# pakozm/lua-mapreduce

Hardware: AMD Instinct MI355X
Metric: words/sec (higher is better)
Workload: dtype u8-text/i64-counts; 1 GPU; model=europarl-wordcount, global_batch=49158635, seq_len=49158635, parallelism=dp1, splits_per_gpu=197, partitions=1, partitioner=hash-mulhi, ingestion=resident-hbm

## Files before the change

mapreduce_amd/ops/hip/mr_kernels.hip:

```cpp

#include "common.h"


#define TOK_BYTES 16

__global__ void tokenize_kernel(const u8* __restrict__ text, long n,
                                u64* __restrict__ out_hash,
                                u64* __restrict__ out_pos,
                                unsigned long long* __restrict__ counter,
                                long cap) {
  long t0 = ((long)blockIdx.x * blockDim.x + threadIdx.x) * (long)TOK_BYTES;
  long stride = (long)gridDim.x * blockDim.x * TOK_BYTES;
  for (long base = t0; base < n; base += stride) {
    long end = base + TOK_BYTES < n ? base + TOK_BYTES : n;
    u8 prev = (base == 0) ? ' ' : text[base - 1];
    for (long i = base; i < end; ++i) {
      u8 c = text[i];
      if (!is_ws(c) && is_ws(prev)) {
        u64 h = FNV64_OFFSET;
        long j = i;
        while (j < n) {
          u8 cc = text[j];
          if (is_ws(cc)) break;
          h ^= cc;
// ... 697 lines not shown
        int lane = threadIdx.x & (WAVE - 1);
        unsigned long long lt_mask =
            (lane == 63) ? ~0ull >> 1 : ((1ull << lane) - 1);
        while (pending) {
          int leader = __ffsll(pending) - 1;
          u64 lead_bk = __shfl(bk, leader, WAVE);
          unsigned long long members =
              __ballot(mine && bk == lead_bk) & pending;
          int nmem = __popcll(members);
          unsigned long long base = 0;
          if (lane == leader)
            base = atomicAdd(&spill_counter[lead_bk],
                             (unsigned long long)nmem);
          base = __shfl(base, leader, WAVE);
          if (members & (1ull << lane)) {
            long r = (long)base + __popcll(members & lt_mask);
            if (r < spill_cap) {
              long o = (long)lead_bk * spill_cap + r;
              out_hash[o] = sh_[wi];
              out_pos[o] = mypos;
            }
          }
          pending &= ~members;
        }
      }
    } else {
      u32 my_ns = (u32)__popc(miss_mask);
      u32 incl = my_ns;
      #pragma unroll
      for (int off = 1; off < WAVE; off <<= 1) {
        u32 x = __shfl_up(incl, off, WAVE);
        if ((threadIdx.x & (WAVE - 1)) >= off) incl += x;
      }
      u32 wave_total = __shfl(incl, WAVE - 1, WAVE);
      int lane = threadIdx.x & (WAVE - 1);
      if (wave_total && (int)wave_total > wleft) {
        for (int i = lane; i < wleft; i += WAVE)
          if (wchunk + i < spill_cap) out_hash[wchunk + i] = HT_EMPTY;
        int grab = (int)wave_total > SPILL_CHUNK ? (int)wave_total
                                                 : SPILL_CHUNK;
        unsigned long long nb = 0;
        if (lane == 0)
          nb = atomicAdd(spill_counter, (unsigned long long)grab);
        wchunk = (long)__shfl(nb, 0, WAVE);
        wleft = grab;
      }
      long o = wchunk + (long)(incl - my_ns);
      if (wave_total) {
        wchunk += wave_total;
        wleft -= (int)wave_total;
      }
      u32 smw = sm0;
      #pragma unroll
      for (int wi = 0; wi < 8; ++wi) {
        if (miss_mask & (1u << wi)) {
          u64 p = v6_spill_pos(wpos0, smw, m32, long_len);
          if (MODE == 4) {
            my_words += sh_[wi] + p + (u64)o;
          } else if (o < spill_cap) {
            out_hash[o] = sh_[wi];
            out_pos[o] = p;
          }
          ++o;
        }
        smw &= smw - 1;
      }
    }
    }
  }
  {
    int lane = threadIdx.x & (WAVE - 1);
    for (int i = lane; i < wleft; i += WAVE)
      if (wchunk + i < spill_cap) out_hash[wchunk + i] = HT_EMPTY;
  }
  __syncthreads();
  for (int s = tid; s < CACHE_N; s += blockDim.x)
    if (ckeys[s] != HT_EMPTY && ccnt[s])
      ht_add(ckeys[s], cpos[s], (i64)ccnt[s], tkeys, tvals, texm, cap_mask);
  unsigned long long ws = my_words;
  for (int off = 32; off > 0; off >>= 1) ws += __shfl_down(ws, off, WAVE);
  if (lane_id() == 0 && ws) atomicAdd(nwords, ws);
}

__global__ __launch_bounds__(256) void tok_ablate_kernel(
    const u8* __restrict__ text, long n, int mode,
    u64* __restrict__ ckeys_g , i64* __restrict__ sink,
    u64* __restrict__ out_hash, u64* __restrict__ out_pos,
    unsigned long long* __restrict__ spill_counter, long spill_cap) {
  __shared__ u8 tile[TOK_TILE + TOK_HALO];
  __shared__ u64 ckeys[TOK_CACHE];
  __shared__ u64 cpos[TOK_CACHE];
  __shared__ u32 ccnt[TOK_CACHE];
  for (int s = threadIdx.x; s < TOK_CACHE; s += blockDim.x) {
    ckeys[s] = HT_EMPTY;
    ccnt[s] = 0;
  }
  unsigned long long acc = 0;
  long tile0 = (long)blockIdx.x * TOK_TILE;
  long tstride = (long)gridDim.x * TOK_TILE;
  for (long base = tile0; base < n; base += tstride) {
    __syncthreads();
    long avail = n - base;
    long want = avail < TOK_TILE + TOK_HALO ? avail : TOK_TILE + TOK_HALO;
    for (int o = threadIdx.x * 16; o < want; o += blockDim.x * 16) {
      if (o + 16 <= want && (((uintptr_t)&text[base + o]) & 15) == 0) {
        *(uint4*)&tile[o] = *(const uint4*)&text[base + o];
      } else {
        for (int b = 0; b < 16 && o + b < want; ++b)
          tile[o + b] = text[base + o + b];
      }
    }
    __syncthreads();
    if (mode == 1) {
      acc += tile[threadIdx.x];
      continue;
    }
    long my0 = (long)threadIdx.x * TOK_BYTES;
    long myend = my0 + TOK_BYTES;
    if (myend > avail) myend = avail;
    if (my0 >= myend) continue;
    u64 sh[8];
    u64 sp[8];
    int ns = 0;
    u8 prev = (base + my0 == 0) ? ' ' : (my0 ? tile[my0 - 1] : text[base - 1]);
    for (long i = my0; i < myend; ++i) {
      u8 c = tile[i];
      if (!is_ws(c) && is_ws(prev)) {
        u64 h = FNV64_OFFSET;
        long j = i;
        if (mode == 2) {
          while (j < want && !is_ws(tile[j])) ++j;
          acc += (u64)(j - i);
        } else {
          while (j < want) {
            u8 cc = tile[j];
            if (is_ws(cc)) break;
            h ^= cc;
            h *= FNV64_PRIME;
            ++j;
          }
          if (j == want && base + j < n) {
            long g = base + j;
            while (g < n && !is_ws(text[g])) {
              h ^= text[g];
              h *= FNV64_PRIME;
              ++g;
            }
            j = g - base;
          }
        }
        if (mode == 3) {
          acc += h;
        } else if (mode >= 4) {
          u64 k = remap_key(h);
          u64 p = ((u64)(base + i) << 16) | (u64)(j - i);
          u32 slot = (u32)((k ^ (k >> 32)) & (TOK_CACHE - 1));
          bool done = false;
          for (int pr = 0; pr < TOK_PROBE; ++pr) {
            u64 cur = ckeys[slot];
            if (cur == k) {
              atomicAdd(&ccnt[slot], 1u);
              done = true;
              break;
            }
            if (cur == HT_EMPTY) {
              u64 prevk = atomicCAS((unsigned long long*)&ckeys[slot],
// ... 385 lines not shown
```

mapreduce_amd/ops/hip/ops_ext.hip:

```cpp

#include <ATen/hip/HIPContext.h>
#include <torch/extension.h>

#include <limits>
#include <map>
#include <mutex>
#include <optional>
#include <utility>

#include "asof.hip"
#include "extract_sorted.hip"
#include "frame.hip"
#include "gradsum.hip"
#include "graph.hip"
#include "group.hip"
#include "join.hip"
#include "lex_order.hip"
#include "mr_kernels.hip"
#include "postings_phrase.hip"
#include "postings_query.hip"
#include "radix_sort.hip"
#include "seg_scan.hip"
#include "token_ordinals.hip"

namespace {

constexpr int kBlock = 256;
constexpr long kMaxBlocks = 2048;

long grid_for(long n, long per_thread = 1) {
  long want = (n + (long)kBlock * per_thread - 1) / ((long)kBlock * per_thread);
  if (want < 1) want = 1;
  return want < kMaxBlocks ? want : kMaxBlocks;
}

hipStream_t cur_stream() { return at::hip::getCurrentHIPStream(); }

constexpr int kTokWavesPerCu = 16;

struct TokOccupancy {
  int blocks_per_cu = 0;
  int cus = 0;
};

TokOccupancy tok_occupancy(const void* kfn, int blockn) {
  static std::mutex mu;
  static std::map<std::pair<const void*, int>, TokOccupancy> cache;
  int dev = 0;
  C10_HIP_CHECK(hipGetDevice(&dev));
  std::lock_guard<std::mutex> lock(mu);
  auto it = cache.find({kfn, dev});
  if (it != cache.end()) return it->second;
  TokOccupancy o;
  C10_HIP_CHECK(hipOccupancyMaxActiveBlocksPerMultiprocessor(
      &o.blocks_per_cu, kfn, blockn, 0));
  C10_HIP_CHECK(hipDeviceGetAttribute(
      &o.cus, hipDeviceAttributeMultiprocessorCount, dev));
  TORCH_CHECK(o.blocks_per_cu > 0 && o.cus > 0,
              "tokenizer occupancy query returned ", o.blocks_per_cu,
              " blocks/CU on ", o.cus, " CUs");
  cache[{kfn, dev}] = o;
  return o;
}

template <typename K>
long tok_grid(K kfn, int blockn, long n, long tile_bytes) {
  long tiles = (n + tile_bytes - 1) / tile_bytes;
  if (tiles < 1) tiles = 1;
  TokOccupancy o = tok_occupancy(reinterpret_cast<const void*>(kfn), blockn);
  int per_cu = kTokWavesPerCu / (blockn / WAVE);
  if (per_cu > o.blocks_per_cu) per_cu = o.blocks_per_cu;
  long resident = (long)per_cu * o.cus;
  long blocks = tiles < resident ? tiles : resident;
  return blocks < kMaxBlocks ? blocks : kMaxBlocks;
}

int rs_items() {
  static int v = -1;
  if (v < 0) {
    const char* e = getenv("MR_RS_ITEMS");
    const char* v1 = getenv("MR_RADIX_V1");
    v = (e && atoi(e) == 4 && !(v1 && v1[0] == '1')) ? 4 : 8;
  }
  return v;
}

long rs_tile() { return (long)RS_BLOCK * rs_items(); }

bool radix_v1_forced() {
  const char* v = getenv("MR_RADIX_V1");
  return v && v[0] == '1';
}

bool radix_v2_forced() {
  static int f = -1;
  if (f < 0) {
    const char* v = getenv("MR_RADIX_V2");
    f = (v && v[0] == '1') ? 1 : 0;
  }
  return f == 1;
}

#define RS_STAGED_SCATTER(VT, SKIP, BT, LATE)                              \
  (radix_v2_forced()                                                       \
       ? (rs_items() == 4 ? radix_scatter_v2_kernel<4, VT, SKIP, BT>       \
                          : radix_scatter_v2_kernel<8, VT, SKIP, BT>)      \
       : (rs_items() == 4 ? radix_scatter_v3_kernel<4, VT, SKIP, BT, LATE> \
                          : radix_scatter_v3_kernel<8, VT, SKIP, BT, LATE>))

void launch_radix_hist(const u64* kin, long n, int shift, long ntiles,
                       i64* hist) {
  auto kfn = rs_items() == 4 ? radix_hist_kernel<4> : radix_hist_kernel<8>;
  hipLaunchKernelGGL(kfn, dim3(ntiles), dim3(RS_BLOCK), 0, cur_stream(),
                     kin, n, shift, ntiles, hist);
}

void launch_radix_scatter(const u64* kin, const u64* vin, long n, int shift,
                          long ntiles, const i64* base, u64* kout,
                          u64* vout) {
  static int use_v1 = -1;
  if (use_v1 < 0) use_v1 = radix_v1_forced() ? 1 : 0;
  if (use_v1)
    hipLaunchKernelGGL(radix_scatter_kernel, dim3(ntiles), dim3(RS_BLOCK), 0,
                       cur_stream(), kin, vin, n, shift, ntiles, base, kout,
                       vout);
  else {
    auto kfn = RS_STAGED_SCATTER(u64, false, i64, true);
    hipLaunchKernelGGL(kfn, dim3(ntiles), dim3(RS_BLOCK),
                       0, cur_stream(), kin, vin, n, shift, ntiles, base,
                       kout, vout);
  }
}

void launch_radix_scatter32(const u64* kin, const u32* vin, long n,
                            int shift, long ntiles, const i64* base,
                            u64* kout, u32* vout) {
  auto kfn = RS_STAGED_SCATTER(u32, false, i64, true);
  hipLaunchKernelGGL(kfn, dim3(ntiles), dim3(RS_BLOCK), 0, cur_stream(),
                     kin, vin, n, shift, ntiles, base, kout, vout);
}

template <bool SKIP>
void launch_bucketize_hist(const u64* kin, long n, int shift, long ntiles,
                           u32* hist) {
  auto kfn = rs_items() == 4 ? radix_hist_kernel<4, SKIP, u32, true>
                             : radix_hist_kernel<8, SKIP, u32, true>;
  if (radix_v2_forced())
    kfn = rs_items() == 4 ? radix_hist_kernel<4, SKIP, u32>
                          : radix_hist_kernel<8, SKIP, u32>;
  hipLaunchKernelGGL(kfn, dim3(ntiles), dim3(RS_BLOCK), 0, cur_stream(),
                     kin, n, shift, ntiles, hist);
}

template <typename VT, bool SKIP>
void launch_bucketize_scatter(const u64* kin, const VT* vin, long n,
                              int shift, long ntiles, const u32* base,
                              u64* kout, VT* vout) {
  auto kfn = RS_STAGED_SCATTER(VT, SKIP, u32, false);
  hipLaunchKernelGGL(kfn, dim3(ntiles), dim3(RS_BLOCK), 0, cur_stream(),
                     kin, vin, n, shift, ntiles, base, kout, vout);
}

u64* u64p(torch::Tensor& t) { return reinterpret_cast<u64*>(t.data_ptr<i64>()); }
const u64* u64cp(const torch::Tensor& t) {
  return reinterpret_cast<const u64*>(t.data_ptr<i64>());
}

void check_dev_i64(const torch::Tensor& t, const char* name) {
  TORCH_CHECK(t.is_cuda(), name, " must be on GPU");
  TORCH_CHECK(t.scalar_type() == torch::kInt64, name, " must be int64");
  TORCH_CHECK(t.is_contiguous(), name, " must be contiguous");
}

}

std::vector<torch::Tensor> tokenize(torch::Tensor text, long cap) {
  TORCH_CHECK(text.is_cuda() && text.scalar_type() == torch::kUInt8 &&
              text.is_contiguous(), "text must be contiguous u8 on GPU");
  long n = text.numel();
  auto opts = torch::TensorOptions().device(text.device()).dtype(torch::kInt64);
  auto out_hash = torch::empty({cap}, opts);
  auto out_pos = torch::empty({cap}, opts);
  auto counter = torch::zeros({1}, opts);
  long blocks = grid_for(n, TOK_BYTES);
  hipLaunchKernelGGL(tokenize_kernel, dim3(blocks), dim3(kBlock), 0,
                     cur_stream(), text.data_ptr<u8>(), n, u64p(out_hash),
                     u64p(out_pos),
                     reinterpret_cast<unsigned long long*>(counter.data_ptr<i64>()),
                     cap);
  return {out_hash, out_pos, counter};
}

void tokenize_count(torch::Tensor text, long pos_base, torch::Tensor tkeys,
                    torch::Tensor tvals, torch::Tensor texm,
                    torch::Tensor nwords) {
  TORCH_CHECK(text.is_cuda() && text.scalar_type() == torch::kUInt8 &&
              text.is_contiguous(), "text must be contiguous u8 on GPU");
  long n = text.numel();
  long cap = tkeys.numel();
  TORCH_CHECK((cap & (cap - 1)) == 0, "table capacity must be a power of 2");
  if (!n) return;
  hipLaunchKernelGGL(tokenize_count_kernel, dim3(grid_for(n, TOK_BYTES)),
                     dim3(kBlock), 0, cur_stream(), text.data_ptr<u8>(), n,
                     (u64)pos_base, u64p(tkeys), tvals.data_ptr<i64>(),
                     texm.numel() ? u64p(texm) : nullptr, (u64)(cap - 1),
                     reinterpret_cast<unsigned long long*>(nwords.data_ptr<i64>()));
}

std::vector<torch::Tensor> tokenize_spill_v2(torch::Tensor text,
                                             long pos_base, long cap) {
  TORCH_CHECK(text.is_cuda() && text.scalar_type() == torch::kUInt8 &&
              text.is_contiguous(), "text must be contiguous u8 on GPU");
  long n = text.numel();
  auto opts = torch::TensorOptions().device(text.device()).dtype(torch::kInt64);
  auto out_hash = torch::empty({cap}, opts);
  auto out_pos = torch::empty({cap}, opts);
  auto counter = torch::zeros({1}, opts);
  auto nwords = torch::zeros({1}, opts);
  if (n) {
    auto dummy = torch::empty({16}, opts);
    hipLaunchKernelGGL((tokenize_v6_kernel<16, false, 4096, 0, true>),
                       dim3(grid_for(n, TOK_BYTES)), dim3(kBlock), 0,
                       cur_stream(), text.data_ptr<u8>(), n, (u64)pos_base,
                       u64p(dummy), dummy.data_ptr<i64>(), nullptr,
                       (u64)15, u64p(out_hash), u64p(out_pos),
                       reinterpret_cast<unsigned long long*>(counter.data_ptr<i64>()),
                       cap,
                       reinterpret_cast<unsigned long long*>(nwords.data_ptr<i64>()),
                       nullptr, (const i64*)nullptr, 0, 0L);
  }
  return {out_hash, out_pos, counter, nwords};
}

std::vector<torch::Tensor> tokenize_spill_composite(
    torch::Tensor text, long pos_base, long cap, torch::Tensor split_off,
    long doc_base) {
  TORCH_CHECK(text.is_cuda() && text.scalar_type() == torch::kUInt8 &&
              text.is_contiguous(), "text must be contiguous u8 on GPU");
  check_dev_i64(split_off, "split_off");
  long n = text.numel();
  auto opts = torch::TensorOptions().device(text.device()).dtype(torch::kInt64);
  auto out_hash = torch::empty({cap}, opts);
  auto out_pos = torch::empty({cap}, opts);
  auto counter = torch::zeros({1}, opts);
  auto nwords = torch::zeros({1}, opts);
  if (n) {
    auto dummy = torch::empty({16}, opts);
    hipLaunchKernelGGL((tokenize_v6_kernel<16, false, 4096, 0, true, true>),
                       dim3(grid_for(n, TOK_BYTES)), dim3(kBlock), 0,
                       cur_stream(), text.data_ptr<u8>(), n, (u64)pos_base,
                       u64p(dummy), dummy.data_ptr<i64>(), nullptr,
                       (u64)15, u64p(out_hash), u64p(out_pos),
                       reinterpret_cast<unsigned long long*>(counter.data_ptr<i64>()),
                       cap,
                       reinterpret_cast<unsigned long long*>(nwords.data_ptr<i64>()),
                       nullptr, split_off.data_ptr<i64>(),
                       (int)split_off.numel(), doc_base);
  }
  return {out_hash, out_pos, counter, nwords};
}

void tokenize_cache_spill_composite(
    torch::Tensor text, long pos_base, torch::Tensor tkeys,
    torch::Tensor tvals, torch::Tensor texm, long spill_cap,
    torch::Tensor nwords, torch::Tensor out_hash, torch::Tensor out_pos,
    torch::Tensor counter, torch::Tensor split_off, long doc_base) {
  TORCH_CHECK(text.is_cuda() && text.scalar_type() == torch::kUInt8 &&
              text.is_contiguous(), "text must be contiguous u8 on GPU");
  check_dev_i64(split_off, "split_off");
  long n = text.numel();
  long cap = tkeys.numel();
  TORCH_CHECK((cap & (cap - 1)) == 0, "table capacity must be a power of 2");
  TORCH_CHECK(out_hash.numel() >= spill_cap && out_pos.numel() >= spill_cap,
              "spill arrays too small");
  if (!n) return;
  auto kfn =
      tokenize_v6_kernel<2048, true, 4096, 0, false, true, 2048, 0, 256>;
  long blocks = tok_grid(kfn, kBlock, n, 4096);
  static torch::Tensor cpos_gc;
  long need = blocks * 2048;
  if (!cpos_gc.defined() || cpos_gc.numel() < need ||
      cpos_gc.device() != text.device())
    cpos_gc = torch::empty({need}, torch::TensorOptions()
                                        .device(text.device())
                                        .dtype(torch::kInt64));
  hipLaunchKernelGGL(
      kfn, dim3(blocks), dim3(kBlock), 0, cur_stream(), text.data_ptr<u8>(), n,
      (u64)pos_base, u64p(tkeys), tvals.data_ptr<i64>(),
      texm.numel() ? u64p(texm) : nullptr, (u64)(cap - 1), u64p(out_hash),
      u64p(out_pos),
      reinterpret_cast<unsigned long long*>(counter.data_ptr<i64>()),
      spill_cap,
      reinterpret_cast<unsigned long long*>(nwords.data_ptr<i64>()),
      u64p(cpos_gc), split_off.data_ptr<i64>(), (int)split_off.numel(),
      doc_base);
}

std::vector<torch::Tensor> tokenize_spill(torch::Tensor text, long pos_base,
                                          long cap) {
  TORCH_CHECK(text.is_cuda() && text.scalar_type() == torch::kUInt8 &&
              text.is_contiguous(), "text must be contiguous u8 on GPU");
  long n = text.numel();
  auto opts = torch::TensorOptions().device(text.device()).dtype(torch::kInt64);
  auto out_hash = torch::empty({cap}, opts);
  auto out_pos = torch::empty({cap}, opts);
  auto counter = torch::zeros({1}, opts);
  if (n)
    hipLaunchKernelGGL(tokenize_spill_kernel, dim3(grid_for(n, TOK_BYTES)),
                       dim3(kBlock), 0, cur_stream(), text.data_ptr<u8>(), n,
                       (u64)pos_base, u64p(out_hash), u64p(out_pos),
                       reinterpret_cast<unsigned long long*>(counter.data_ptr<i64>()),
                       cap);
  return {out_hash, out_pos, counter};
}

void tokenize_cache_spill(
    torch::Tensor text, long pos_base, torch::Tensor tkeys,
    torch::Tensor tvals, torch::Tensor texm, long spill_cap,
    torch::Tensor nwords, torch::Tensor out_hash, torch::Tensor out_pos,
    torch::Tensor counter) {
  TORCH_CHECK(text.is_cuda() && text.scalar_type() == torch::kUInt8 &&
              text.is_contiguous(), "text must be contiguous u8 on GPU");
  long n = text.numel();
  long cap = tkeys.numel();
  TORCH_CHECK((cap & (cap - 1)) == 0, "table capacity must be a power of 2");
  TORCH_CHECK(out_hash.numel() >= spill_cap && out_pos.numel() >= spill_cap,
              "spill arrays too small");
  if (n) {
    const char* v = getenv("MR_TOKENIZE_V5");
    const char* v4 = getenv("MR_TOKENIZE_V4");
    if (!(v && v[0] == '1') && !(v4 && v4[0] == '1')) {
      const char* cs = getenv("MR_TOK_CACHE");
      int cache = cs ? atoi(cs) : 2048;
      const char* gp = getenv("MR_TOK_GPOS");
      bool gpos = !(gp && gp[0] == '0');
      const char* ts = getenv("MR_TOK_TILE");
      int tsz = ts ? atoi(ts) : 4096;
      const char* sc = getenv("MR_SPILL_CHUNK");
      int schunk = sc ? atoi(sc) : 2048;
      const char* tb = getenv("MR_TOK_BLOCK");
      int blockn = (tb && atoi(tb) == 512) ? 512 : 256;
      if (blockn == 512) tsz = 8192;
      auto kfn = tokenize_v6_kernel<2048, false, 4096>;
      if (gpos && blockn == 512)
        kfn = tokenize_v6_kernel<2048, true, 8192, 0, false, false, 2048,
                                 0, 512>;
      else if (gpos && tsz == 8192) kfn = tokenize_v6_kernel<2048, true, 8192>;
      else if (gpos && cache == 4096) kfn = tokenize_v6_kernel<4096, true, 4096>;
      else if (gpos && cache == 1024) kfn = tokenize_v6_kernel<1024, true, 4096>;
      else if (gpos && schunk == 128)
        kfn = tokenize_v6_kernel<2048, true, 4096, 0, false, false, 128>;
      else if (gpos && schunk == 1024)
        kfn = tokenize_v6_kernel<2048, true, 4096, 0, false, false, 1024>;
      else if (gpos && schunk == 2048)
        kfn = tokenize_v6_kernel<2048, true, 4096, 0, false, false, 2048>;
      else if (gpos && schunk == 4096)
        kfn = tokenize_v6_kernel<2048, true, 4096, 0, false, false, 4096>;
      else if (gpos) kfn = tokenize_v6_kernel<2048, true, 4096>;
      else if (cache == 512) kfn = tokenize_v6_kernel<512, false, 4096>;
      else if (cache == 1024) kfn = tokenize_v6_kernel<1024, false, 4096>;
      else if (schunk == 128)
        kfn = tokenize_v6_kernel<2048, false, 4096, 0, false, false, 128>;
      long blocks = tok_grid(kfn, blockn, n, tsz);
      static torch::Tensor cpos_g;
      u64* cpg = nullptr;
      if (gpos) {
        long need = blocks * (cache > 2048 ? cache : 2048);
        if (!cpos_g.defined() || cpos_g.numel() < need ||
            cpos_g.device() != text.device())
          cpos_g = torch::empty({need},
                                torch::TensorOptions().device(text.device())
                                    .dtype(torch::kInt64));
        cpg = u64p(cpos_g);
      }
      hipLaunchKernelGGL(kfn,
                         dim3(blocks), dim3(blockn), 0,
                         cur_stream(), text.data_ptr<u8>(), n, (u64)pos_base,
                         u64p(tkeys), tvals.data_ptr<i64>(),
                         texm.numel() ? u64p(texm) : nullptr, (u64)(cap - 1),
                         u64p(out_hash), u64p(out_pos),
                         reinterpret_cast<unsigned long long*>(counter.data_ptr<i64>()),
                         spill_cap,
                         reinterpret_cast<unsigned long long*>(nwords.data_ptr<i64>()),
                         cpg, (const i64*)nullptr, 0, 0L);
    } else if (!(v && v[0] == '1'))
      hipLaunchKernelGGL(tokenize_cache_spill_kernel,
                         dim3(grid_for(n, TOK_BYTES)), dim3(kBlock), 0,
                         cur_stream(), text.data_ptr<u8>(), n, (u64)pos_base,
                         u64p(tkeys), tvals.data_ptr<i64>(),
                         texm.numel() ? u64p(texm) : nullptr, (u64)(cap - 1),
                         u64p(out_hash), u64p(out_pos),
                         reinterpret_cast<unsigned long long*>(counter.data_ptr<i64>()),
                         spill_cap,
                         reinterpret_cast<unsigned long long*>(nwords.data_ptr<i64>()));
    else
      hipLaunchKernelGGL(tokenize_v5_kernel,
                         dim3(grid_for(n, TOK_BYTES)), dim3(kBlock), 0,
                         cur_stream(), text.data_ptr<u8>(), n, (u64)pos_base,
                         u64p(tkeys), tvals.data_ptr<i64>(),
                         texm.numel() ? u64p(texm) : nullptr, (u64)(cap - 1),
                         u64p(out_hash), u64p(out_pos),
                         reinterpret_cast<unsigned long long*>(counter.data_ptr<i64>()),
                         spill_cap,
                         reinterpret_cast<unsigned long long*>(nwords.data_ptr<i64>()));
  }
}

void tokenize_cache_spill_bucketed(
    torch::Tensor text, long pos_base, torch::Tensor tkeys,
    torch::Tensor tvals, torch::Tensor texm, long spill_bcap,
    torch::Tensor nwords, torch::Tensor out_hash, torch::Tensor out_pos,
    torch::Tensor counters) {
  TORCH_CHECK(text.is_cuda() && text.scalar_type() == torch::kUInt8 &&
              text.is_contiguous(), "text must be contiguous u8 on GPU");
  long n = text.numel();
  long cap = tkeys.numel();
  TORCH_CHECK((cap & (cap - 1)) == 0, "table capacity must be a power of 2");
  TORCH_CHECK(counters.numel() >= 256, "counters must hold 256 buckets");
  TORCH_CHECK(out_hash.numel() >= 256 * spill_bcap &&
              out_pos.numel() >= 256 * spill_bcap, "spill arrays too small");
  if (!n) return;
  const char* gp = getenv("MR_TOK_GPOS");
  bool gpos = !(gp && gp[0] == '0');
  auto kfn = tokenize_v6_kernel<2048, false, 4096, 0, false, false, 512, 256>;
  if (gpos)
    kfn = tokenize_v6_kernel<2048, true, 4096, 0, false, false, 512, 256>;
  long blocks = tok_grid(kfn, kBlock, n, 4096);
  static torch::Tensor cpos_gb;
  u64* cpg = nullptr;
  if (gpos) {
    long need = blocks * 2048;
    if (!cpos_gb.defined() || cpos_gb.numel() < need ||
        cpos_gb.device() != text.device())
      cpos_gb = torch::empty({need},
                             torch::TensorOptions().device(text.device())
                                 .dtype(torch::kInt64));
    cpg = u64p(cpos_gb);
  }
  hipLaunchKernelGGL(kfn, dim3(blocks), dim3(kBlock), 0, cur_stream(),
                     text.data_ptr<u8>(), n, (u64)pos_base, u64p(tkeys),
                     tvals.data_ptr<i64>(),
                     texm.numel() ? u64p(texm) : nullptr, (u64)(cap - 1),
                     u64p(out_hash), u64p(out_pos),
                     reinterpret_cast<unsigned long long*>(counters.data_ptr<i64>()),
                     spill_bcap,
                     reinterpret_cast<unsigned long long*>(nwords.data_ptr<i64>()),
// ... 1259 lines not shown

namespace {
static_assert(GRAPH_BLOCK == SEG_SCAN_BLOCK,
              "the graph kernels are launched by SEG_SCAN_LAUNCH");

void check_graph_f64(const torch::Tensor& t, const torch::Tensor& like,
                     long n, const char* name) {
  TORCH_CHECK(t.is_cuda(), name, " must be on GPU");
  TORCH_CHECK(t.scalar_type() == torch::kFloat64, name, " must be float64");
  TORCH_CHECK(t.is_contiguous(), name, " must be contiguous");
  TORCH_CHECK(t.device() == like.device(), name,
              " must be on the device of sums");
  TORCH_CHECK(t.numel() == n, name, " must hold ", n, " entries, got ",
              t.numel());
}
}

torch::Tensor graph_propagate(torch::Tensor offsets, torch::Tensor src,
                              torch::Tensor x, long op, bool f64) {
  check_dev_i64(offsets, "offsets");
  check_dev_i64(x, "x");
  TORCH_CHECK(src.is_cuda(), "src must be on GPU");
  TORCH_CHECK(src.scalar_type() == torch::kInt32, "src must be int32");
  TORCH_CHECK(src.is_contiguous(), "src must be contiguous");
  TORCH_CHECK(offsets.device() == x.device() && src.device() == x.device(),
              "offsets, src and x must be on the same device");
  long n = x.numel(), m = src.numel();
  TORCH_CHECK(offsets.numel() == n + 1, "offsets must hold ", n + 1,
              " entries, got ", offsets.numel());
  TORCH_CHECK(n < (1L << 31) && m < (1L << 31),
              "graph ops take fewer than 2^31 edges and rows, got ", m,
              " and ", n);
  TORCH_CHECK(op >= SEG_SUM && op <= SEG_MAX,
              "op must be 0 (sum), 1 (min) or 2 (max), got ", op);
  TORCH_CHECK(op == SEG_SUM || !f64, "graph min / max take int64 values");
  const i64 ident = op == SEG_SUM ? 0
                    : op == SEG_MIN ? std::numeric_limits<i64>::max()
                                    : std::numeric_limits<i64>::min();
  auto out = torch::full({n}, ident, x.options());
  if (!n || !m) return out;
  long ntiles = (m + GRAPH_TILE - 1) / GRAPH_TILE;
  auto tf = torch::empty({ntiles}, x.options());
  auto ta = torch::empty({ntiles}, x.options());
  auto lr = torch::empty({ntiles}, x.options());
  auto la = torch::empty({ntiles}, x.options());
  SEG_SCAN_LAUNCH(graph_tile_kernel, ntiles, offsets.data_ptr<i64>(),
                  src.data_ptr<int>(), u64cp(x), n, m, u64p(out),
                  tf.data_ptr<i64>(), u64p(ta), lr.data_ptr<i64>(), u64p(la));
  auto c = seg_scan_carry(tf, ta, op, f64);
  SEG_SCAN_LAUNCH(graph_lead_kernel, grid_for(ntiles), lr.data_ptr<i64>(),
                  u64cp(la), c[0].data_ptr<i64>(), u64cp(c[1]), ntiles, n,
                  u64p(out));
  return out;
}

std::vector<torch::Tensor> pagerank_update(torch::Tensor sums,
                                           torch::Tensor old,
                                           torch::Tensor inv_out,
                                           double damping,
                                           torch::Tensor dangling) {
  long n = sums.numel();
  check_graph_f64(sums, sums, n, "sums");
  check_graph_f64(old, sums, n, "old");
  check_graph_f64(inv_out, sums, n, "inv_out");
  check_graph_f64(dangling, sums, 1, "dangling");
  TORCH_CHECK(n < (1L << 31), "graph ops take fewer than 2^31 rows, got ", n);
  auto nw = torch::empty({n}, sums.options());
  auto contrib = torch::empty({n}, sums.options());
  long blocks = n ? grid_for(n) : 0;
  if (blocks > GRAPH_PR_BLOCKS) blocks = GRAPH_PR_BLOCKS;
  auto partials = torch::empty({blocks, 2}, sums.options());
  if (blocks)
    hipLaunchKernelGGL(pagerank_update_kernel, dim3(blocks),
                       dim3(GRAPH_BLOCK), 0, cur_stream(),
                       sums.data_ptr<double>(), old.data_ptr<double>(),
                       inv_out.data_ptr<double>(), n, damping,
                       dangling.data_ptr<double>(), nw.data_ptr<double>(),
                       contrib.data_ptr<double>(),
                       partials.data_ptr<double>());
  return {nw, contrib, partials};
}

py::dict tokenizer_occupancy() {
  auto kfn = tokenize_v6_kernel<2048, true, 4096, 0, false, false, 2048>;
  TokOccupancy o = tok_occupancy(reinterpret_cast<const void*>(kfn), kBlock);
  hipFuncAttributes fa;
  C10_HIP_CHECK(hipFuncGetAttributes(&fa, reinterpret_cast<const void*>(kfn)));
  py::dict d;
  d["blocks_per_cu"] = o.blocks_per_cu;
  d["cus"] = o.cus;
  d["num_regs"] = fa.numRegs;
  d["lds_bytes"] = (long)fa.sharedSizeBytes;
  return d;
}

PYBIND11_MODULE(TORCH_EXTENSION_NAME, m) {
  m.def("group_caps", &group_caps, "(TILE, QMAX) of the group kernels");
  m.def("group_rank_max", &group_rank_max,
        "longest segment of the tile kernel's rank-counting pass");
  m.def("group_order_keys", &group_order_keys,
        "u64 order key of each i64 / f64 value");
  m.def("group_tile_sort", &group_tile_sort,
        "values ordered inside every segment that fits one tile");
  m.def("group_tile_sort_perm", &group_tile_sort_perm,
        "group_tile_sort plus the input row of every value");
  m.def("seg_scan_caps", &seg_scan_caps,
        "(TILE, CARRY_CHUNK) of the segmented scan");
  m.def("scan_by_key_sorted", &scan_by_key_sorted,
        "inclusive sum/min/max scan within runs of equal keys");
  m.def("seg_scan_reduce", &seg_scan_reduce,
        "pass 1 of scan_by_key_sorted: per-tile (flags, aggregate)");
  m.def("seg_scan_carry", &seg_scan_carry,
        "pass 2 of scan_by_key_sorted: per-tile carry-in");
  m.def("seg_scan_apply", &seg_scan_apply,
        "pass 3 of scan_by_key_sorted: the running column");
  m.def("session_flags", &session_flags,
        "1 where a row starts a key or follows a gap in time");
  m.def("graph_caps", &graph_caps,
        "(TILE, PR_BLOCKS) of the graph kernels");
  m.def("graph_propagate", &graph_propagate,
        "sum / min / max over every row's in-edges of a gathered column");
  m.def("pagerank_update", &pagerank_update,
        "one PageRank update -> (new, contrib, partials)");
  m.def("frame_caps", &frame_caps,
        "(TILE, WIN, RTILE) of the frame kernels");
  m.def("frame_bounds", &frame_bounds, py::arg("keys"), py::arg("times"),
        py::arg("preceding"), py::arg("following"), py::arg("row") = false,
        "range frames of (key, time)-sorted rows -> (lo, hi)");
  m.def("frame_reduce", &frame_reduce,
        "sum / min / max of a value column over per-row frames");
  m.def("frame_tile", &frame_tile,
        "frame_reduce pass 1: (pre, suf, tile aggregates)");
  m.def("frame_tree", &frame_tree,
        "frame_reduce pass 2: the tree over the tile aggregates");
  m.def("frame_apply", &frame_apply,
        "frame_reduce pass 3: one range query per row");
  m.def("group_pick", &group_pick,
        "values at exact rank fractions of each ordered segment");
  m.def("group_distinct_flags", &group_distinct_flags,
        "1 where a row starts a segment or a new value");
  m.def("join_bounds", &join_bounds, py::arg("lkeys"), py::arg("rkeys"),
        py::arg("window") = true,
        "(lo, cnt) of each left key in the sorted right keys");
  m.def("join_bounds_caps", &join_bounds_caps,
        "(BTILE, WIN) of the windowed join_bounds");
  m.def("join_expand", &join_expand,
        "(li, ri) row pairs from the bounds and their exclusive cumsum");
  m.def("join_caps", &join_caps, "(TILE, LDS_ROWS) of join_expand");
  m.def("asof_sorted", &asof_sorted, py::arg("lkeys"), py::arg("ltimes"),
        py::arg("rkeys"), py::arg("rtimes"), py::arg("direction") = 0,
        py::arg("tolerance") = py::none(), py::arg("allow_exact") = true,
        py::arg("f64") = false, py::arg("row") = false,
        "matched right row (or -1) of each left row of two sorted relations");
  m.def("asof_caps", &asof_caps, "(TILE, WIN) of the windowed asof_sorted");
  m.def("tokenizer_occupancy", &tokenizer_occupancy,
        "blocks/CU, registers and static LDS of the default tokenizer");
  m.def("postings_search", &postings_search,
        "ranked AND/OR top-k over the inverted index, one block per query");
  m.def("postings_search_caps", &postings_search_caps,
        "(TMAX, KMAX, BUF) of postings_search");
  m.def("postings_phrase", &postings_phrase,
        "exact-phrase top-k over the positional index, one block per query");
  m.def("token_ordinals", &token_ordinals,
        "(doc, token ordinal within doc) of each occurrence");
  m.def("token_ordinals_caps", &token_ordinals_caps,
        "(GRANULE) of token_ordinals");
  m.def("lex_chunk_keys", &lex_chunk_keys,
        "big-endian 8-byte chunk d of each string as a sortable u64");
  m.def("lex_refine", &lex_refine,
        "(seg, key) head flags + unfinished-string flags");
  m.def("lex_lower_bound", &lex_lower_bound,
        "binary search of byte-string queries in a lex permutation");
  m.def("radix_sort_idx32", &radix_sort_idx32,
        "sort u64 keys with a u32 iota payload -> (keys, perm)");
  m.def("gather_by_u32", &gather_by_u32, "out[i] = vals[idx[i]] (u32 idx)");
  m.def("tokenize", &tokenize, "tokenize text -> (hash, pos, count)");
  m.def("tokenize_count", &tokenize_count,
        "fused tokenize + hash-table count");
  m.def("tokenize_spill_composite", &tokenize_spill_composite,
        "spill-all with fused (word,doc) composite keys");
  m.def("tokenize_cache_spill_composite", &tokenize_cache_spill_composite,
        "composite keys with the LDS cache (misses spill)");
  m.def("tokenize_spill_v2", &tokenize_spill_v2,
        "spill-all tokenizer (chunk-padded; filter HT_EMPTY)");
  m.def("tokenize_spill", &tokenize_spill,
        "tokenize -> compact (hash,pos) arrays");
  m.def("tokenize_cache_spill", &tokenize_cache_spill,
        "tokenize; LDS cache counts the head, misses spill");
  m.def("tokenize_cache_spill_bucketed", &tokenize_cache_spill_bucketed,
        "tokenize; misses spill directly into per-top-byte-bucket regions");
  m.def("tok_ablate", &tok_ablate, "ablation timing (diagnosis)");
  m.def("tok6_ablate", &tok6_ablate, "v6 ablation timing");
  m.def("bucket_count", &bucket_count,
        "LDS count of bucket-partitioned (hash,pos)");
  m.def("hash_insert_count", &hash_insert_count);
  m.def("hash_insert_sum_i64", &hash_insert_sum_i64);
  m.def("hash_extract", &hash_extract);
  m.def("hash_extract_v2", &hash_extract_v2,
        "chunked compaction (HT_EMPTY-padded; mask/trim downstream)");
  m.def("extract_sorted", &extract_sorted,
        "table -> (packed keys|counts|lens, pos, offs, host meta), sorted");
  m.def("extract_sorted_caps", &extract_sorted_caps,
        "(RANK_M, SCAN_TILE) of extract_sorted");
  m.def("head_flags", &head_flags);
  m.def("seg_reduce_i64", &seg_reduce_i64);
  m.def("seg_reduce_i64_minmax", &seg_reduce_i64_minmax);
  m.def("seg_reduce_f64_minmax", &seg_reduce_f64_minmax);
  m.def("seg_first_u64", &seg_first_u64);
  m.def("seg_reduce_f64", &seg_reduce_f64);
  m.def("partition_hist", &partition_hist);
  m.def("pos_len", &pos_len);
  m.def("gather_bytes", &gather_bytes);
  m.def("radix_sort_pairs", &radix_sort_pairs);
  m.def("radix_sort_caps", &radix_sort_caps,
        "(tile records, direct scatter 0/1) of this process's radix sorts");
  m.def("radix_pass", &radix_pass);
  m.def("radix_bucketize", &radix_bucketize, py::arg("keys"),
        py::arg("vals"), py::arg("shift"), py::arg("skip_empty") = false,
        "one-digit partition with native scan -> (keys, vals, bucket_off)");
  m.def("grad_colsum", &grad_colsum, "sum G gradient rows -> D (K6)");
}
```

Measured before the change: 48.12 billion words/s.

## Add v7 tokenizer with register-prefetched next tile and route tokenize paths to it

Adds a tokenize_v7 kernel that stages a 4 KB tile into LDS and, while hashing the current tile, prefetches the next tile into registers, then writes it to LDS after the cache/probe work. Each thread processes 16 bytes with bitmask word-start detection and register-resident hashing. The cache-spill, spill-all and composite entry points now launch v7 by default, with v6 still available through an env var. The change also adds an optional max_blocks grid cap, tuned launch bounds and a debug query for the body used. The aim is to hide global-load latency behind compute, at the cost of more registers and a possibly different occupancy.

Result: faster. 50.28 billion words/s, median of 6 (+4.5%).

```diff
diff --git a/mapreduce_amd/ops/hip/mr_kernels.hip b/mapreduce_amd/ops/hip/mr_kernels.hip
--- a/mapreduce_amd/ops/hip/mr_kernels.hip
+++ b/mapreduce_amd/ops/hip/mr_kernels.hip
@@ -803,6 +803,258 @@
   if (lane_id() == 0 && ws) atomicAdd(nwords, ws);
 }
 
+#define V7_WAIT_VM0 0x0F70
+constexpr int V7_BLOCK = 256;
+
+template <int TILE_N>
+__device__ __forceinline__ void v7_stage_plain(u8* tile,
+                                               const u8* __restrict__ text,
+                                               long base, long want,
+                                               bool aligned) {
+  for (int o = threadIdx.x * 16; o < want; o += V7_BLOCK * 16) {
+    if (aligned && o + 16 <= want) {
+      *(uint4*)&tile[o] = *(const uint4*)&text[base + o];
+    } else {
+      for (int b = 0; b < 16 && o + b < want; ++b)
+        tile[o + b] = text[base + o + b];
+    }
+  }
+}
+
+template <int CACHE_N, bool GPOS, bool SPILL_ALL = false,
+          bool COMPOSITE = false, int SCHUNK = 512>
+__global__ __launch_bounds__(V7_BLOCK, GPOS || SPILL_ALL ? 5 : 3)
+void tokenize_v7_kernel(
+    const u8* __restrict__ text, long n, u64 pos_base,
+    u64* __restrict__ tkeys, i64* __restrict__ tvals, u64* __restrict__ texm,
+    u64 cap_mask, u64* __restrict__ out_hash, u64* __restrict__ out_pos,
+    unsigned long long* __restrict__ spill_counter, long spill_cap,
+    unsigned long long* __restrict__ nwords, u64* __restrict__ cpos_g,
+    const i64* __restrict__ split_off = nullptr, int nsplit_off = 0,
+    long doc_base = 0) {
+  constexpr int TILE_N = V7_BLOCK * TOK_BYTES;
+  __shared__ __align__(16) u8 tile[TILE_N + TOK_HALO];
+  __shared__ u64 ckeys[CACHE_N];
+  __shared__ u64 cpos_l[GPOS ? 1 : CACHE_N];
+  __shared__ u32 ccnt[CACHE_N];
+  u64* cpos = GPOS ? &cpos_g[(u64)blockIdx.x * CACHE_N] : cpos_l;
+  for (int s = threadIdx.x; s < CACHE_N; s += blockDim.x) {
+    ckeys[s] = HT_EMPTY;
+    ccnt[s] = 0;
+  }
+  const int tid = threadIdx.x;
+  const int lane = tid & (WAVE - 1);
+  unsigned long long my_words = 0;
+  constexpr int SPILL_CHUNK = SCHUNK;
+  long wchunk = -1;
+  int wleft = 0;
+  const long tile0 = (long)blockIdx.x * TILE_N;
+  const long tstride = (long)gridDim.x * TILE_N;
+  const bool aligned = (((uintptr_t)text) & 15) == 0;
+  if (tile0 < n) {
+    long avail0 = n - tile0;
+    v7_stage_plain<TILE_N>(tile, text, tile0,
+                           avail0 < TILE_N + TOK_HALO ? avail0
+                                                      : TILE_N + TOK_HALO,
+                           aligned);
+  }
+  const long my0 = (long)tid * TOK_BYTES;
+  u32 pb_cur = (tid == 0 && tile0 > 0 && tile0 < n) ? text[tile0 - 1] : 0x20;
+  __builtin_amdgcn_s_waitcnt(V7_WAIT_VM0);
+  for (long base = tile0; base < n; base += tstride) {
+    const long avail = n - base;
+    const long want = avail < TILE_N + TOK_HALO ? avail : TILE_N + TOK_HALO;
+    const long nbase = base + tstride;
+    const bool pf_fast = aligned && nbase + TILE_N + TOK_HALO <= n;
+    uint4 pf = uint4{0, 0, 0, 0};
+    u32 ph = 0;
+    u32 pb_next = 0x20;
+    if (tid == 0 && nbase < n) pb_next = text[nbase - 1];
+    if (pf_fast) {
+      pf = *(const uint4*)&text[nbase + my0];
+      if (tid < TOK_HALO / 4) ph = *(const u32*)&text[nbase + TILE_N + tid * 4];
+    }
+    __syncthreads();
+    const bool wactive = my0 < avail;
+    const uint4 va = wactive ? *(const uint4*)&tile[my0] : uint4{0, 0, 0, 0};
+    const uint4 vb = wactive ? *(const uint4*)&tile[my0 + 16] : uint4{0, 0, 0, 0};
+    u32 prevb = (base + my0 == 0)
+                    ? 1u
+                    : (wactive ? (u32)is_ws(my0 ? tile[my0 - 1]
+                                                : (u8)pb_cur) : 1u);
+    __syncthreads();
+    const u64 q0 = (u64)va.x | ((u64)va.y << 32);
+    const u64 q1 = (u64)va.z | ((u64)va.w << 32);
+    const u64 q2 = (u64)vb.x | ((u64)vb.y << 32);
+    const u64 q3 = (u64)vb.z | ((u64)vb.w << 32);
+    u32 m32 = ws_mask8(q0) | (ws_mask8(q1) << 8) |
+              (ws_mask8(q2) << 16) | (ws_mask8(q3) << 24);
+    long lim32 = want - my0;
+    if (lim32 < 32)
+      m32 |= (lim32 <= 0) ? 0xFFFFFFFFu : ~((1u << lim32) - 1);
+    u32 sm = wactive ? (~m32 & ((m32 << 1) | prevb) & 0xFFFFu) : 0u;
+    long limw = avail - my0;
+    if (limw < 16) sm &= (limw <= 0) ? 0u : ((1u << limw) - 1);
+    my_words += __popc(sm);
+    u64 sh_[8];
+    const u32 sm0 = sm;
+    u32 long_len = 0;
+    const u64 wpos0 = pos_base + (u64)(base + my0);
+    u32 miss_mask = 0;
+    #pragma unroll
+    for (int wi = 0; wi < 8; ++wi) {
+      if (!sm) break;
+      int s = __ffs(sm) - 1;
+      sm &= sm - 1;
+      u32 t = m32 >> s;
+      u64 h = FNV64_OFFSET;
+      u32 len;
+      if (t) {
+        len = (u32)(__ffs(t) - 1);
+        {
+          const int di = s >> 2;
+          const u32 bsh = (u32)s & 3u;
+          u32 a0 = (di & 2) ? ((di & 1) ? va.w : va.z) : ((di & 1) ? va.y : va.x);
+          u32 a1 = (di & 2) ? ((di & 1) ? vb.x : va.w) : ((di & 1) ? va.z : va.y);
+          u32 a2 = (di & 2) ? ((di & 1) ? vb.y : vb.x) : ((di & 1) ? va.w : va.z);
+          u64 w = (u64)__builtin_amdgcn_alignbyte(a1, a0, bsh) |
+                  ((u64)__builtin_amdgcn_alignbyte(a2, a1, bsh) << 32);
+          u32 nb = len < 8 ? len : 8;
+          w &= ~(u64)0 >> (64 - 8 * nb);
+          h = whash_chunk(h, w);
+        }
+        for (u32 c = 8; c < len; c += 8) {
+          int j0 = s + (int)c;
+          int qi = j0 >> 3;
+          u64 lo = (qi & 2) ? ((qi & 1) ? q3 : q2) : ((qi & 1) ? q1 : q0);
+          u64 hi = (qi >= 3) ? 0 : ((qi & 2) ? q3 : ((qi & 1) ? q2 : q1));
+          int sh2 = 8 * (j0 & 7);
+          u64 w = sh2 ? ((lo >> sh2) | (hi << (64 - sh2))) : lo;
+          u32 rem = len - c;
+          if (rem < 8) w &= (((u64)1 << (8 * rem)) - 1);
+          h = whash_chunk(h, w);
+        }
+        h = whash_fin(h, len);
+      } else {
+        long g = base + my0 + s;
+        u64 chunk = 0;
+        int cb = 0;
+        long wlen = 0;
+        while (g < n && !is_ws(text[g])) {
+          chunk |= (u64)text[g] << (8 * cb);
+          if (++cb == 8) {
+            h = whash_chunk(h, chunk);
+            chunk = 0;
+            cb = 0;
+          }
+          ++g;
+          ++wlen;
+        }
+        if (cb) h = whash_chunk(h, chunk);
+        h = whash_fin(h, (u64)wlen);
+        len = (u32)(wlen > 0xFFFF ? 0xFFFF : wlen);
+        long_len = len;
+      }
+      if (COMPOSITE) {
+        i64 byte = (i64)(pos_base + (u64)(base + my0 + s));
+        int doc = ub_minus1(split_off, nsplit_off, byte);
+        h ^= splitmix64_dev((u64)(doc + doc_base));
+      }
+      u64 k = remap_key(h);
+      sh_[wi] = k;
+      if (SPILL_ALL) {
+        miss_mask |= 1u << wi;
+        continue;
+      }
+      u64 p = ((pos_base + (u64)(base + my0 + s)) << 16) | (u64)len;
+      u32 slot = (u32)((k ^ (k >> 32)) & (CACHE_N - 1));
+      bool done = false;
+      for (int pr = 0; pr < TOK_PROBE; ++pr) {
+        u64 cur2 = ckeys[slot];
+        if (cur2 == k) {
+          atomicAdd(&ccnt[slot], 1u);
+          done = true;
+          break;
+        }
+        if (cur2 == HT_EMPTY) {
+          u64 prevk = atomicCAS((unsigned long long*)&ckeys[slot],
+                                (unsigned long long)HT_EMPTY,
+                                (unsigned long long)k);
+          if (prevk == HT_EMPTY) cpos[slot] = p;
+          if (prevk == HT_EMPTY || prevk == k) {
+            atomicAdd(&ccnt[slot], 1u);
+            done = true;
+            break;
+          }
+        }
+        slot = (slot + 1) & (CACHE_N - 1);
+      }
+      if (!done) miss_mask |= 1u << wi;
+    }
+    if (nbase < n) {
+      if (pf_fast) {
+        *(uint4*)&tile[my0] = pf;
+        if (tid < TOK_HALO / 4) *(u32*)&tile[TILE_N + tid * 4] = ph;
+      } else {
+        long navail = n - nbase;
+        v7_stage_plain<TILE_N>(tile, text, nbase,
+                               navail < TILE_N + TOK_HALO ? navail
+                                                          : TILE_N + TOK_HALO,
+                               aligned);
+      }
+    }
+    pb_cur = pb_next;
+    {
+      u32 my_ns = (u32)__popc(miss_mask);
+      u32 incl = my_ns;
+      #pragma unroll
+      for (int off = 1; off < WAVE; off <<= 1) {
+        u32 x = __shfl_up(incl, off, WAVE);
+        if (lane >= off) incl += x;
+      }
+      u32 wave_total = __shfl(incl, WAVE - 1, WAVE);
+      if (wave_total && (int)wave_total > wleft) {
+        for (int i = lane; i < wleft; i += WAVE)
+          if (wchunk + i < spill_cap) out_hash[wchunk + i] = HT_EMPTY;
+        int grab = (int)wave_total > SPILL_CHUNK ? (int)wave_total
+                                                 : SPILL_CHUNK;
+        unsigned long long nb = 0;
+        if (lane == 0)
+          nb = atomicAdd(spill_counter, (unsigned long long)grab);
+        wchunk = (long)__shfl(nb, 0, WAVE);
+        wleft = grab;
+      }
+      long o = wchunk + (long)(incl - my_ns);
+      if (wave_total) {
+        wchunk += wave_total;
+        wleft -= (int)wave_total;
+      }
+      u32 smw = sm0;
+      #pragma unroll
+      for (int wi = 0; wi < 8; ++wi) {
+        if (miss_mask & (1u << wi)) {
+          u64 p = v6_spill_pos(wpos0, smw, m32, long_len);
+          if (o < spill_cap) {
+            out_hash[o] = sh_[wi];
+            out_pos[o] = p;
+          }
+          ++o;
+        }
+        smw &= smw - 1;
+      }
+    }
+  }
+  for (int i = lane; i < wleft; i += WAVE)
+    if (wchunk + i < spill_cap) out_hash[wchunk + i] = HT_EMPTY;
+  __syncthreads();
+  for (int s = tid; s < CACHE_N; s += blockDim.x)
+    if (ckeys[s] != HT_EMPTY && ccnt[s])
+      ht_add(ckeys[s], cpos[s], (i64)ccnt[s], tkeys, tvals, texm, cap_mask);
+  unsigned long long ws = my_words;
+  for (int off = 32; off > 0; off >>= 1) ws += __shfl_down(ws, off, WAVE);
+  if (lane == 0 && ws) atomicAdd(nwords, ws);
+}
+
 __global__ __launch_bounds__(256) void tok_ablate_kernel(
     const u8* __restrict__ text, long n, int mode,
     u64* __restrict__ ckeys_g , i64* __restrict__ sink,
diff --git a/mapreduce_amd/ops/hip/ops_ext.hip b/mapreduce_amd/ops/hip/ops_ext.hip
--- a/mapreduce_amd/ops/hip/ops_ext.hip
+++ b/mapreduce_amd/ops/hip/ops_ext.hip
@@ -101,6 +101,26 @@
   return f == 1;
 }
 
+bool tok_v6_forced() {
+  static int f = -1;
+  if (f < 0) {
+    const char* v = getenv("MR_TOKENIZE_V6");
+    f = (v && v[0] == '1') ? 1 : 0;
+  }
+  return f == 1;
+}
+
+static_assert(kBlock == V7_BLOCK, "v7 launches use kBlock threads");
+
+const char* g_tok_last_body = "none";
+
+long tok_cap_blocks(long blocks, long max_blocks) {
+  if (max_blocks == 0) return blocks;
+  long m = max_blocks < 1 ? 1 : (max_blocks > kMaxBlocks ? kMaxBlocks
+                                                         : max_blocks);
+  return blocks < m ? blocks : m;
+}
+
 #define RS_STAGED_SCATTER(VT, SKIP, BT, LATE)                              \
   (radix_v2_forced()                                                       \
        ? (rs_items() == 4 ? radix_scatter_v2_kernel<4, VT, SKIP, BT>       \
@@ -208,7 +228,8 @@
 }
 
 std::vector<torch::Tensor> tokenize_spill_v2(torch::Tensor text,
-                                             long pos_base, long cap) {
+                                             long pos_base, long cap,
+                                             long max_blocks) {
   TORCH_CHECK(text.is_cuda() && text.scalar_type() == torch::kUInt8 &&
               text.is_contiguous(), "text must be contiguous u8 on GPU");
   long n = text.numel();
@@ -219,8 +240,12 @@
   auto nwords = torch::zeros({1}, opts);
   if (n) {
     auto dummy = torch::empty({16}, opts);
-    hipLaunchKernelGGL((tokenize_v6_kernel<16, false, 4096, 0, true>),
-                       dim3(grid_for(n, TOK_BYTES)), dim3(kBlock), 0,
+    auto kfn = tokenize_v7_kernel<16, false, true>;
+    if (tok_v6_forced()) kfn = tokenize_v6_kernel<16, false, 4096, 0, true>;
+    g_tok_last_body = tok_v6_forced() ? "v6" : "v7";
+    hipLaunchKernelGGL(kfn,
+                       dim3(tok_cap_blocks(grid_for(n, TOK_BYTES), max_blocks)),
+                       dim3(kBlock), 0,
                        cur_stream(), text.data_ptr<u8>(), n, (u64)pos_base,
                        u64p(dummy), dummy.data_ptr<i64>(), nullptr,
                        (u64)15, u64p(out_hash), u64p(out_pos),
@@ -234,7 +259,7 @@
 
 std::vector<torch::Tensor> tokenize_spill_composite(
     torch::Tensor text, long pos_base, long cap, torch::Tensor split_off,
-    long doc_base) {
+    long doc_base, long max_blocks) {
   TORCH_CHECK(text.is_cuda() && text.scalar_type() == torch::kUInt8 &&
               text.is_contiguous(), "text must be contiguous u8 on GPU");
   check_dev_i64(split_off, "split_off");
@@ -246,8 +271,13 @@
   auto nwords = torch::zeros({1}, opts);
   if (n) {
     auto dummy = torch::empty({16}, opts);
-    hipLaunchKernelGGL((tokenize_v6_kernel<16, false, 4096, 0, true, true>),
-                       dim3(grid_for(n, TOK_BYTES)), dim3(kBlock), 0,
+    auto kfn = tokenize_v7_kernel<16, false, true, true>;
+    if (tok_v6_forced())
+      kfn = tokenize_v6_kernel<16, false, 4096, 0, true, true>;
+    g_tok_last_body = tok_v6_forced() ? "v6" : "v7";
+    hipLaunchKernelGGL(kfn,
+                       dim3(tok_cap_blocks(grid_for(n, TOK_BYTES), max_blocks)),
+                       dim3(kBlock), 0,
                        cur_stream(), text.data_ptr<u8>(), n, (u64)pos_base,
                        u64p(dummy), dummy.data_ptr<i64>(), nullptr,
                        (u64)15, u64p(out_hash), u64p(out_pos),
@@ -264,7 +294,8 @@
     torch::Tensor text, long pos_base, torch::Tensor tkeys,
     torch::Tensor tvals, torch::Tensor texm, long spill_cap,
     torch::Tensor nwords, torch::Tensor out_hash, torch::Tensor out_pos,
-    torch::Tensor counter, torch::Tensor split_off, long doc_base) {
+    torch::Tensor counter, torch::Tensor split_off, long doc_base,
+    long max_blocks) {
   TORCH_CHECK(text.is_cuda() && text.scalar_type() == torch::kUInt8 &&
               text.is_contiguous(), "text must be contiguous u8 on GPU");
   check_dev_i64(split_off, "split_off");
@@ -274,9 +305,11 @@
   TORCH_CHECK(out_hash.numel() >= spill_cap && out_pos.numel() >= spill_cap,
               "spill arrays too small");
   if (!n) return;
-  auto kfn =
-      tokenize_v6_kernel<2048, true, 4096, 0, false, true, 2048, 0, 256>;
-  long blocks = tok_grid(kfn, kBlock, n, 4096);
+  auto kfn = tokenize_v7_kernel<2048, true, false, true, 2048>;
+  if (tok_v6_forced())
+    kfn = tokenize_v6_kernel<2048, true, 4096, 0, false, true, 2048, 0, 256>;
+  g_tok_last_body = tok_v6_forced() ? "v6" : "v7";
+  long blocks = tok_cap_blocks(tok_grid(kfn, kBlock, n, 4096), max_blocks);
   static torch::Tensor cpos_gc;
   long need = blocks * 2048;
   if (!cpos_gc.defined() || cpos_gc.numel() < need ||
@@ -318,7 +351,7 @@
     torch::Tensor text, long pos_base, torch::Tensor tkeys,
     torch::Tensor tvals, torch::Tensor texm, long spill_cap,
     torch::Tensor nwords, torch::Tensor out_hash, torch::Tensor out_pos,
-    torch::Tensor counter) {
+    torch::Tensor counter, long max_blocks) {
   TORCH_CHECK(text.is_cuda() && text.scalar_type() == torch::kUInt8 &&
               text.is_contiguous(), "text must be contiguous u8 on GPU");
   long n = text.numel();
@@ -361,7 +394,14 @@
       else if (cache == 1024) kfn = tokenize_v6_kernel<1024, false, 4096>;
       else if (schunk == 128)
         kfn = tokenize_v6_kernel<2048, false, 4096, 0, false, false, 128>;
-      long blocks = tok_grid(kfn, blockn, n, tsz);
+      g_tok_last_body = "v6";
+      if (!tok_v6_forced() && cache == 2048 && tsz == 4096 &&
+          schunk == 2048 && blockn == V7_BLOCK) {
+        if (gpos) kfn = tokenize_v7_kernel<2048, true, false, false, 2048>;
+        else kfn = tokenize_v7_kernel<2048, false>;
+        g_tok_last_body = "v7";
+      }
+      long blocks = tok_cap_blocks(tok_grid(kfn, blockn, n, tsz), max_blocks);
       static torch::Tensor cpos_g;
       u64* cpg = nullptr;
       if (gpos) {
@@ -1787,7 +1827,9 @@
 }
 
 py::dict tokenizer_occupancy() {
-  auto kfn = tokenize_v6_kernel<2048, true, 4096, 0, false, false, 2048>;
+  auto kfn = tokenize_v7_kernel<2048, true, false, false, 2048>;
+  if (tok_v6_forced())
+    kfn = tokenize_v6_kernel<2048, true, 4096, 0, false, false, 2048>;
   TokOccupancy o = tok_occupancy(reinterpret_cast<const void*>(kfn), kBlock);
   hipFuncAttributes fa;
   C10_HIP_CHECK(hipFuncGetAttributes(&fa, reinterpret_cast<const void*>(kfn)));
@@ -1796,10 +1838,15 @@
   d["cus"] = o.cus;
   d["num_regs"] = fa.numRegs;
   d["lds_bytes"] = (long)fa.sharedSizeBytes;
+  d["body"] = tok_v6_forced() ? "v6" : "v7";
   return d;
 }
 
+std::string tokenizer_last_body() { return g_tok_last_body; }
+
 PYBIND11_MODULE(TORCH_EXTENSION_NAME, m) {
+  m.def("tokenizer_last_body", &tokenizer_last_body,
+        "body of the last v6/v7 tokenizer launch: v7, v6 or none");
   m.def("group_caps", &group_caps, "(TILE, QMAX) of the group kernels");
   m.def("group_rank_max", &group_rank_max,
         "longest segment of the tile kernel's rank-counting pass");
@@ -1883,14 +1930,26 @@
   m.def("tokenize_count", &tokenize_count,
         "fused tokenize + hash-table count");
   m.def("tokenize_spill_composite", &tokenize_spill_composite,
+        py::arg("text"), py::arg("pos_base"), py::arg("cap"),
+        py::arg("split_off"), py::arg("doc_base"), py::arg("max_blocks") = 0,
         "spill-all with fused (word,doc) composite keys");
   m.def("tokenize_cache_spill_composite", &tokenize_cache_spill_composite,
+        py::arg("text"), py::arg("pos_base"), py::arg("tkeys"),
+        py::arg("tvals"), py::arg("texm"), py::arg("spill_cap"),
+        py::arg("nwords"), py::arg("out_hash"), py::arg("out_pos"),
+        py::arg("counter"), py::arg("split_off"), py::arg("doc_base"),
+        py::arg("max_blocks") = 0,
         "composite keys with the LDS cache (misses spill)");
-  m.def("tokenize_spill_v2", &tokenize_spill_v2,
+  m.def("tokenize_spill_v2", &tokenize_spill_v2, py::arg("text"),
+        py::arg("pos_base"), py::arg("cap"), py::arg("max_blocks") = 0,
         "spill-all tokenizer (chunk-padded; filter HT_EMPTY)");
   m.def("tokenize_spill", &tokenize_spill,
         "tokenize -> compact (hash,pos) arrays");
-  m.def("tokenize_cache_spill", &tokenize_cache_spill,
+  m.def("tokenize_cache_spill", &tokenize_cache_spill, py::arg("text"),
+        py::arg("pos_base"), py::arg("tkeys"), py::arg("tvals"),
+        py::arg("texm"), py::arg("spill_cap"), py::arg("nwords"),
+        py::arg("out_hash"), py::arg("out_pos"), py::arg("counter"),
+        py::arg("max_blocks") = 0,
         "tokenize; LDS cache counts the head, misses spill");
   m.def("tokenize_cache_spill_bucketed", &tokenize_cache_spill_bucketed,
         "tokenize; misses spill directly into per-top-byte-bucket regions");
```
